# trzy/FasterRCNN

Measured on AMD Instinct MI355X. Metric: images/sec (600x1000) Faster-RCNN VGG-16 inference, higher is better.
Workload: dtype f32 (float32 tensors and accumulation; 15 GEMM layers in the f32x3 split-operand emulation = two fp16 terms per block-scaled operand, three fp16 MFMAs per product; 0 in f32x6 = three bf16 terms, six bf16 MFMAs; the other 2 on exact-f32 MFMA; strict exact-f32 everywhere: config.strict_f32_images_per_

## Files before the change

fasterrcnn_amd/_native.py:

```python
import ctypes as C
import os

_HERE = os.path.dirname(os.path.abspath(__file__))
LIB_PATH = os.environ.get("FRCNN_LIB_PATH") or os.path.join(_HERE, "csrc", "libfrcnn_hip.so")

OK = 0
ABI_VERSION = 21
ERRORS = {0: "FRCNN_OK", -1: "FRCNN_EINVAL", -2: "FRCNN_EHIP", -3: "FRCNN_ENOMEM",
          -4: "FRCNN_EUNSUPPORTED", -5: "FRCNN_ENODEVICE"}
RELU = 1
POOL2 = 2
NUM_KCLASS = 11
KCLASS_NAMES = ("conv3x3_mfma", "conv3x3_c3", "linear_mfma", "proposals", "roi_pool", "other", "winograd_transforms",
                "winograd_gemm", "winograd_x6_transforms", "winograd_x6_gemm", "winograd_x3f")

SYMBOLS = (
    "frcnn_abi_version", "frcnn_error_string", "frcnn_last_hip_error", "frcnn_device_count",
    "frcnn_anchors", "frcnn_pack_conv3x3", "frcnn_pack_conv3x3_c3", "frcnn_pack_fc_chw_to_hwc",
    "frcnn_pack_stack_rows", "frcnn_conv3x3_c3", "frcnn_conv3x3_c3_cmax", "frcnn_conv3x3_workspace_bytes", "frcnn_conv3x3_nhwc",
    "frcnn_maxpool2x2_nhwc",
    "frcnn_linear_workspace_bytes", "frcnn_linear", "frcnn_softmax_rows", "frcnn_rpn_proposals",
    "frcnn_nms", "frcnn_roi_pool", "frcnn_roi_pool_x3t", "frcnn_detections", "frcnn_ctx_create", "frcnn_ctx_create_proposals", "frcnn_ctx_destroy",
    "frcnn_ctx_bytes", "frcnn_vgg16_forward", "frcnn_ctx_tensor", "frcnn_ctx_timing_enable",
    "frcnn_ctx_timing_read",
    "frcnn_output_block_layout", "frcnn_stream_depend", "frcnn_ctx_submit_stats", "frcnn_predict_submit", "frcnn_streams_share_queue",
    "frcnn_fold_bn_pack", "frcnn_conv_workspace_bytes", "frcnn_conv_nhwc", "frcnn_conv_nhwc_math", "frcnn_conv_nhwc_x3g", "frcnn_conv_nhwc_x3g_tickets", "frcnn_pack_conv_x3g_weights", "frcnn_x3_saturation_events", "frcnn_tensor_absmax", "frcnn_conv7x7_s2_c3",
    "frcnn_maxpool3x3_s2_nhwc", "frcnn_spatial_mean_nhwc", "frcnn_resnet_forward", "frcnn_rpn_targets",
    "frcnn_preprocess_workspace_bytes", "frcnn_preprocess",
    "frcnn_conv3x3_uses_winograd", "frcnn_resnet_block_uses_winograd", "frcnn_pack_conv3x3_winograd",
    "frcnn_pack_conv3x3_winograd_taps", "frcnn_conv3x3_winograd_workspace_bytes",
    "frcnn_conv3x3_nhwc_winograd",
    "frcnn_conv3x3_uses_winograd_fused", "frcnn_resnet_block_uses_winograd_fused", "frcnn_pack_conv3x3_winograd_fused", "frcnn_pack_conv3x3_winograd_fused_taps",
    "frcnn_conv3x3_nhwc_winograd_fused",
    "frcnn_roi_align", "frcnn_roi_align_backward",
    "frcnn_x6t_record_bytes", "frcnn_split_rows_x6t", "frcnn_gemm_x6t_workspace_bytes", "frcnn_gemm_x6t", "frcnn_split_pixels_x6t", "frcnn_split_patches3x3_x6t",
    "frcnn_conv3x3_uses_winograd_x6", "frcnn_conv3x3_winograd_x6_pack_bytes", "frcnn_pack_conv3x3_winograd_x6",
    "frcnn_conv3x3_winograd_x6_workspace_bytes", "frcnn_conv3x3_nhwc_winograd_x6",
    "frcnn_pixel_absmax", "frcnn_split_pixels_x3t", "frcnn_split_patches3x3_x3t",
    "frcnn_x3t_blob_bytes", "frcnn_pack_rows_x3t", "frcnn_conv3x3_winograd_x3_pack_bytes", "frcnn_pack_conv3x3_winograd_x3",
    "frcnn_conv3x3_winograd_x3_workspace_bytes", "frcnn_conv3x3_nhwc_winograd_x3",
    "frcnn_conv3x3_winograd_x3_fused_workspace_bytes", "frcnn_conv3x3_nhwc_winograd_x3_fused", "frcnn_conv3x3_nhwc_winograd_x3_chain",
    "frcnn_x3t_record_bytes", "frcnn_rows_scale_x3t", "frcnn_split_rows_x3t", "frcnn_gemm_x3t_workspace_bytes", "frcnn_gemm_x3t",
    "frcnn_conv3x3_nhwc_winograd_fused_maps", "frcnn_ctx_create_backbone", "frcnn_resnet_backbone", "frcnn_resnet_forward_features", "frcnn_resnet_rpn_roipool", "frcnn_ctx_create_head", "frcnn_resnet_head",
    "frcnn_label_proposals", "frcnn_gather_rows", "frcnn_rpn_loss", "frcnn_detector_loss",
    "frcnn_gemm_tn_math", "frcnn_conv3x3_wgrad_math", "frcnn_conv_wgrad_math", "frcnn_bottleneck_backward_workspace_bytes", "frcnn_bottleneck_backward",
    "frcnn_gemm_tn_workspace_bytes", "frcnn_gemm_tn", "frcnn_conv3x3_wgrad_workspace_bytes", "frcnn_conv3x3_wgrad",
    "frcnn_pack_conv3x3_dgrad", "frcnn_relu_backward", "frcnn_dropout", "frcnn_dropout_relu_backward", "frcnn_add_inplace", "frcnn_maxpool2x2_backward",
    "frcnn_roi_pool_backward_workspace_bytes", "frcnn_roi_pool_backward", "frcnn_transpose", "frcnn_sgd_step", "frcnn_sgd_step_fold",
    "frcnn_conv_wgrad_workspace_bytes", "frcnn_conv_wgrad", "frcnn_conv_dgrad_workspace_bytes", "frcnn_conv_dgrad", "frcnn_conv_dgrad_math",
    "frcnn_pack_conv_dgrad", "frcnn_scale_rows", "frcnn_bn_scale_shift", "frcnn_spatial_mean_backward",
    "frcnn_ops_roi_align", "frcnn_ops_roi_align_backward", "frcnn_ops_roi_pool", "frcnn_ops_roi_pool_backward",
    "frcnn_ops_nms_workspace_bytes", "frcnn_ops_nms",
    "frcnn_ops_ms_roi_align", "frcnn_ops_ms_roi_align_workspace_bytes", "frcnn_ops_ms_roi_align_backward",
    "frcnn_ops_half_run", "frcnn_ops_roi_align_16", "frcnn_ops_roi_align_backward_16", "frcnn_ops_roi_pool_16",
    "frcnn_ops_roi_pool_backward_16", "frcnn_ops_ms_roi_align_16", "frcnn_ops_ms_roi_align_backward_16",
    "frcnn_ops_ps_roi_pool", "frcnn_ops_ps_roi_pool_backward", "frcnn_ops_ps_roi_align", "frcnn_ops_ps_roi_align_backward",
    "frcnn_ops_ps_roi_pool_16", "frcnn_ops_ps_roi_pool_backward_16", "frcnn_ops_ps_roi_align_16", "frcnn_ops_ps_roi_align_backward_16",
    "frcnn_ops_deform_workspace_bytes", "frcnn_ops_deform_forward", "frcnn_ops_deform_backward_columns", "frcnn_ops_deform_backward_offset",
    "frcnn_ops_deform_input_plan", "frcnn_ops_deform_backward_input", "frcnn_ops_deform_backward_weight",
    "frcnn_ops_deform_roi_pool_cull_list", "frcnn_ops_deform_roi_pool_workspace_bytes", "frcnn_ops_deform_roi_pool",
    "frcnn_ops_deform_roi_pool_backward", "frcnn_ops_deform_roi_pool_16", "frcnn_ops_deform_roi_pool_backward_16",
    "frcnn_ops_box_iou_rotated", "frcnn_ops_nms_rotated", "frcnn_ops_roi_align_rotated_cull_list", "frcnn_ops_roi_align_rotated",
    "frcnn_ops_roi_align_rotated_backward", "frcnn_ops_roi_align_rotated_16", "frcnn_ops_roi_align_rotated_backward_16",
    "frcnn_ops_diff_iou_rotated", "frcnn_ops_diff_iou_rotated_backward",
    "frcnn_ops_soft_nms_block_threads", "frcnn_ops_soft_nms_lds_boxes", "frcnn_ops_soft_nms_max_boxes", "frcnn_ops_soft_nms_workspace_bytes",
# ... 304 lines not shown
    "frcnn_maxpool3x3_s2_nhwc": (C.c_int, [_vp, _vp, _i, _i, _i, _vp]),
    "frcnn_spatial_mean_nhwc": (C.c_int, [_vp, _vp, _i, _i, _i, _i, _vp]),
    "frcnn_resnet_forward": (C.c_int, [_vp, C.POINTER(ResNetWeights), C.POINTER(ForwardParams), _vp, _i, _i,
                                       _vp, _vp, _vp, _vp, _vp, _vp, _vp]),
    "frcnn_resnet_forward_features": (C.c_int, [_vp, C.POINTER(ResNetWeights), C.POINTER(ForwardParams), _vp, _i, _i,
                                                _vp, _vp, _vp, _vp, _vp, _vp, _vp]),
    "frcnn_resnet_backbone": (C.c_int, [_vp, C.POINTER(ResNetWeights), C.POINTER(ForwardParams), _vp, _i, _i, _i, _vp, _vp]),
    "frcnn_pixel_absmax": (C.c_int, [_vp, _vp, C.c_longlong, _i, _vp]),
    "frcnn_split_pixels_x3t": (C.c_int, [_vp, _vp, _vp, _vp, _i, _i, _i, _i, _i, _i, _vp]),
    "frcnn_split_patches3x3_x3t": (C.c_int, [_vp, _vp, _vp, _vp, _i, _i, _i, _i, _i, _i, _vp]),
    "frcnn_x3t_blob_bytes": (C.c_size_t, [_i, _i, _i]),
    "frcnn_pack_rows_x3t": (C.c_int, [_vp, _i, _sz, _vp, _i, _i, _i, _i, _vp]),
    "frcnn_conv3x3_winograd_x3_pack_bytes": (C.c_size_t, [_i, _i]),
    "frcnn_pack_conv3x3_winograd_x3": (C.c_int, [_vp, _vp, _i, _i, _vp]),
    "frcnn_conv3x3_winograd_x3_workspace_bytes": (C.c_size_t, [_i, _i, _i, _i, _i]),
    "frcnn_conv3x3_nhwc_winograd_x3": (C.c_int, [_vp, _vp, _vp, _vp, _i, _i, _i, _i, _i, _u, _vp, _sz, _vp]),
    "frcnn_conv3x3_winograd_x3_fused_workspace_bytes": (C.c_size_t, [_i, _i, _i]),
    "frcnn_conv3x3_nhwc_winograd_x3_fused": (C.c_int, [_vp, _vp, _vp, _vp, _i, _i, _i, _i, _i, _u, _vp, _sz, _vp]),
    "frcnn_conv3x3_nhwc_winograd_x3_chain": (C.c_int, [_vp, _vp, _vp, _vp, _i, _i, _i, _i, _i, _u, _i, _vp, _sz, _vp, _vp, _vp]),
    "frcnn_x3t_record_bytes": (C.c_size_t, [_i, _i]),
    "frcnn_rows_scale_x3t": (C.c_int, [_vp, _i, _sz, _vp, _i, _i, _i, _i, _vp]),
    "frcnn_split_rows_x3t": (C.c_int, [_vp, _i, _sz, _vp, _vp, _i, _i, _i, _i, _vp]),
    "frcnn_gemm_x3t_workspace_bytes": (C.c_size_t, [_i, _i, _i, _i]),
    "frcnn_gemm_x3t": (C.c_int, [_vp, _vp, _i, _sz, _sz, _vp, _vp, _i, _sz, _sz, _vp, _vp, _vp, _i, _sz, _i, _i, _i, _i, _u, _vp, _sz, _vp]),
    "frcnn_ctx_create_backbone": (C.c_int, [C.POINTER(C.c_void_p), _i, _i, _i]),
    "frcnn_ctx_create_head": (C.c_int, [C.POINTER(C.c_void_p), _i]),
    "frcnn_resnet_rpn_roipool": (C.c_int, [_vp, C.POINTER(ResNetWeights), C.POINTER(ForwardParams), _vp, _i, _i, _vp, _vp, _vp, _vp, _vp, _vp]),
    "frcnn_resnet_head": (C.c_int, [_vp, C.POINTER(ResNetWeights), C.POINTER(ForwardParams), _vp, _i, _vp, _vp, _vp]),
    "frcnn_conv3x3_nhwc_winograd_fused_maps": (C.c_int, [_vp, _vp, _vp, _vp, _i, _i, _i, _i, _i, _u, _vp]),
    "frcnn_label_proposals": (C.c_int, [_vp, _vp, _i, _vp, _vp, _i, _i, _f, _f, C.POINTER(C.c_float), C.POINTER(C.c_float),
                                        _vp, _vp, _vp, _vp, _vp, _vp]),
    "frcnn_gather_rows": (C.c_int, [_vp, _vp, _i, _i, _vp, _vp]),
    "frcnn_rpn_loss": (C.c_int, [_vp, _i, _i, _vp, _i, _vp, _vp, _vp, _vp]),
    "frcnn_detector_loss": (C.c_int, [_vp, _vp, _vp, _vp, _i, _i, _vp, _vp, _i, _vp]),
    "frcnn_gemm_tn_workspace_bytes": (C.c_size_t, [_i, _i, _i]),
    "frcnn_gemm_tn": (C.c_int, [_vp, _i, _vp, _i, _vp, _i, _i, _i, _i, _vp, _sz, _vp]),
    "frcnn_gemm_tn_math": (C.c_int, [_vp, _i, _vp, _i, _vp, _i, _i, _i, _i, _i, _vp, _sz, _vp]),
    "frcnn_conv3x3_wgrad_math": (C.c_int, [_vp, _vp, _vp, _i, _i, _i, _i, _i, _vp, _sz, _vp]),
    "frcnn_conv_wgrad_math": (C.c_int, [_vp, _vp, _vp, _i, _i, _i, _i, _i, _i, _i, _i, _i, _vp, _sz, _vp]),
    "frcnn_bottleneck_backward_workspace_bytes": (C.c_int, [_vp, _vp, _vp, _vp, _i, _i, _i, _i, _i, C.POINTER(C.c_size_t), C.POINTER(C.c_size_t)]),
    "frcnn_bottleneck_backward": (C.c_int, [_vp, _vp, _vp, _vp, _vp, _vp, _vp, _vp, _vp, _vp, _vp, _vp, _vp, _i, _i, _i, _i, _i, _i, _vp, _sz, _vp, _sz,
                                            _vp, _vp]),
    "frcnn_conv3x3_wgrad_workspace_bytes": (C.c_size_t, [_i, _i, _i, _i]),
    "frcnn_conv3x3_wgrad": (C.c_int, [_vp, _vp, _vp, _i, _i, _i, _i, _vp, _sz, _vp]),
    "frcnn_pack_conv3x3_dgrad": (C.c_int, [_vp, _vp, _i, _i, _vp]),
    "frcnn_conv_wgrad_workspace_bytes": (C.c_size_t, [_i] * 8),
# ... 96 lines not shown
```

fasterrcnn_amd/csrc/api.hip:

```cpp
#include "common.h"
#include <algorithm>
#include <cmath>
#include <cstring>
#include <initializer_list>
#include <string>
#include <vector>
#include <new>

namespace frcnn {

static thread_local std::string g_hip_error;
void set_hip_error(hipError_t e) { g_hip_error = hipGetErrorString(e); }

static size_t align_up(size_t v, size_t a) { return (v + a - 1) / a * a; }

struct EventRec { int cls; hipEvent_t start, stop; };

struct Scratch {
    void* p = nullptr;
    size_t bytes = 0;
    int reserve(size_t want, hipStream_t s, bool zero)
    {
        if (want <= bytes) return FRCNN_OK;
        if (p) { FRCNN_HIP_TRY(hipStreamSynchronize(s)); release(); }
// ... 308 lines not shown
    if (!d_a || !d_inv_scale) return FRCNN_EINVAL;
    return launch_rows_scale_x3t(d_a, lda, a_batch_floats, d_inv_scale, rows, rows_padded, K, batches, as_stream(stream));
}

int frcnn_split_rows_x3t(const float* d_a, int lda, size_t a_batch_floats, const float* d_inv_scale, void* d_rec, int rows, int rows_padded,
                         int K, int batches, void* stream)
{
    if (!d_a || !d_rec || !d_inv_scale) return FRCNN_EINVAL;
    return launch_split_rows_x3t(d_a, lda, a_batch_floats, d_inv_scale, d_rec, rows, rows_padded, K, batches, as_stream(stream));
}

size_t frcnn_gemm_x3t_workspace_bytes(int M, int N, int K, int batches) { return gemm_x3t_workspace_bytes(M, N, K, batches); }

int frcnn_gemm_x3t(const void* d_a_rec, const float* d_a_inv, int a_rows, size_t a_batch_bytes, size_t a_inv_batch_floats,
                   const void* d_b_rec, const float* d_b_inv, int b_rows, size_t b_batch_bytes, size_t b_inv_batch_floats,
                   const float* d_bias, const float* d_residual, float* d_c, int ldc, size_t c_batch_floats, int M, int N, int K,
                   int batches, unsigned flags, void* d_ws, size_t ws_bytes, void* stream)
{
    return launch_gemm_x3t(d_a_rec, d_a_inv, a_rows, a_batch_bytes, a_inv_batch_floats, d_b_rec, d_b_inv, b_rows, b_batch_bytes,
                           b_inv_batch_floats, d_bias, d_residual, d_c, ldc, c_batch_floats, M, N, K, batches, flags, d_ws, ws_bytes,
                           as_stream(stream));
}

size_t frcnn_conv3x3_winograd_x3_fused_workspace_bytes(int n_maps, int H, int W)
{
    return n_maps > 0 && H > 0 && W > 0 ? conv3x3_winograd_x3_fused_workspace_bytes(n_maps, H, W) : 0;
}

int frcnn_conv3x3_nhwc_winograd_x3_fused(const float* d_x, const void* d_blob, const float* d_bias, float* d_y, int n_maps, int H, int W,
                                         int cin, int cout, unsigned flags, void* d_ws, size_t ws_bytes, void* stream)
{
    if (!d_x || !d_blob || !d_bias || !d_y) return FRCNN_EINVAL;
    return launch_conv3x3_winograd_x3_fused(d_x, d_blob, d_bias, d_y, n_maps, H, W, cin, cout, flags, d_ws, ws_bytes, as_stream(stream));
}

int frcnn_pixel_absmax(const float* d_x, float* d_cmax, long long pixels, int c, void* stream)
{
    if (!d_x || !d_cmax) return FRCNN_EINVAL;
    return launch_pixel_absmax(d_x, d_cmax, pixels, c, as_stream(stream));
}

int frcnn_split_pixels_x3t(const float* d_x, const float* d_cmax, void* d_rec, float* d_inv_scale, int n_maps, int H, int W, int c, int stride,
                           int rows_padded, void* stream)
{
    if (!d_x || !d_rec) return FRCNN_EINVAL;
    return launch_split_pixels_x3t(d_x, d_cmax, d_rec, d_inv_scale, n_maps, H, W, c, stride, rows_padded, as_stream(stream));
// ... 1582 lines not shown
```

fasterrcnn_amd/csrc/common.h:

```cpp
#pragma once
#include <hip/hip_runtime.h>
#include <stdint.h>
#include <stddef.h>
#include <stdlib.h>
#include "../../include/frcnn_hip.h"

typedef float f32x4  __attribute__((ext_vector_type(4)));
typedef float f32x16 __attribute__((ext_vector_type(16)));

inline const char* frcnn_knob(const char* name)
{
#ifdef FRCNN_EXPERIMENT_KNOBS
    return getenv(name);
#else
    (void)name;
    return nullptr;
#endif
}

namespace frcnn {

void set_hip_error(hipError_t e);

inline int check_launch() {
// ... 108 lines not shown
size_t gemm_x6t_workspace_bytes(int M, int N, int K, int batches);
void gemm_x6t_set_tiles(int mode);
int launch_gemm_x6t(const void* a_rec, int a_rows, size_t a_batch_bytes, const void* b_rec, int b_rows, size_t b_batch_bytes,
                    const float* bias, const float* residual, float* c, int ldc, size_t c_batch_floats, int M, int N, int K, int batches,
                    unsigned flags, void* ws, size_t ws_bytes, hipStream_t s, int tiles_mode = -1);
int launch_split_pixels_x6t(const float* x, void* rec, int N, int H, int W, int C, int stride, int rows_padded, hipStream_t s);
int gemm_x6t_get_tiles();
int launch_gemm_x6t_reduce(const float* ws, const float* bias, const float* residual, float* c, int ldc, size_t c_batch_floats, int M, int N,
                           int batches, int splits, int relu, hipStream_t s);
size_t x3t_record_bytes(int rows_padded, int K);
int launch_rows_scale_x3t(const float* a, int lda, size_t a_batch_floats, float* inv_scale, int R, int rows_padded, int K, int batches,
                          hipStream_t s);
int launch_split_rows_x3t(const float* a, int lda, size_t a_batch_floats, const float* inv_scale, void* rec, int R, int rows_padded, int K,
                          int batches, hipStream_t s);
int launch_split_pixels_x3t(const float* x, const float* cmax, void* rec, float* inv, int N, int H, int W, int C, int stride, int rows_padded,
                            hipStream_t s);
int launch_split_patches3x3_x3t(const float* x, const float* cmax, void* rec, float* inv, int N, int H, int W, int C, int stride,
                                int rows_padded, hipStream_t s);
size_t gemm_x3t_workspace_bytes(int M, int N, int K, int batches);
int launch_gemm_x3t(const void* a_rec, const float* a_inv, int a_rows, size_t a_batch_bytes, size_t a_inv_batch, const void* b_rec,
                    const float* b_inv, int b_rows, size_t b_batch_bytes, size_t b_inv_batch, const float* bias, const float* residual,
                    float* c, int ldc, size_t c_batch_floats, int M, int N, int K, int batches, unsigned flags, void* ws, size_t ws_bytes,
                    hipStream_t s, int tiles_mode = -1);
size_t x3t_blob_bytes(int rows_padded, int K, int batches);
int launch_pack_rows_x3t(const float* a, int lda, size_t a_batch_floats, void* blob, int R, int rows_padded, int K, int batches, hipStream_t s);
int launch_pixel_absmax(const float* x, float* cmax, long long pixels, int C, hipStream_t s);
size_t conv3x3_winograd_x3_pack_bytes(int cout, int cin);
int launch_pack_conv3x3_winograd_x3(const float* u_f32, void* ublob, int cout, int cin, hipStream_t s);
size_t conv3x3_winograd_x3_workspace_bytes(int N, int H, int W, int cin, int cout);
int winograd_x3_plan(int N, int H, int W, int cin, int cout, unsigned flags, void* ws, size_t ws_bytes, void** V, float** vinv, float** cmax,
                     float** M, void** G, size_t* g_bytes);
int launch_winograd_x3_input(const float* x, float* cmax, void* vrec, float* vinv, int N, int H, int W, int cin, hipStream_t s,
                             const float* cmax_ready = nullptr);
int launch_winograd_x3_gemm(const void* vrec, const float* vinv, const void* ublob, float* M, int N, int H, int W, int cin, int cout, void* gws,
                            size_t gws_bytes, hipStream_t s);
int launch_conv3x3_winograd_x3(const float* x, const void* ublob, const float* b, float* y, int N, int H, int W, int cin, int cout,
                               unsigned flags, void* ws, size_t ws_bytes, hipStream_t s,
                               const float* cmax_ready = nullptr, float* cmax_out = nullptr);
size_t conv3x3_winograd_x3_fused_workspace_bytes(int N, int H, int W);
int launch_conv3x3_winograd_x3_fused(const float* x, const void* ublob, const float* b, float* y, int N, int H, int W, int cin, int cout,
                                     unsigned flags, void* ws, size_t ws_bytes, hipStream_t s, const float* cmax_ready = nullptr,
                                     float* cmax_out = nullptr);
int launch_roi_pool_x3t(const float* fm, int fh, int fw, int c, const float* rois, const int32_t* n_rois, int max_rois, int pooled,
                        float scale, float* cmax, float* inv, void* rec, int rec_rows, hipStream_t s, bool cmax_ready = false);
bool conv3x3_uses_winograd_x6(int cin, int cout);
size_t conv3x3_winograd_x6_pack_bytes(int cout, int cin);
// ... 98 lines not shown
```

fasterrcnn_amd/csrc/gemm_x3t.hip:

```cpp
#include "x3t.h"

namespace frcnn {

typedef _Float16 hx_f16x8 __attribute__((ext_vector_type(8)));

#ifndef HX_ABLATE
#define HX_ABLATE 0
#endif
__global__ __launch_bounds__(256)
void rows_scale_x3t_kernel(const float* __restrict__ a, int lda, size_t a_batch, float* __restrict__ inv_scale, int R, int rows_padded,
                           int K, int batches)
{
    const int lane = threadIdx.x & 63;
    const long long wave = (long long)blockIdx.x * 4 + (threadIdx.x >> 6);
    if (wave >= (long long)batches * rows_padded) return;
    const int row = (int)(wave % rows_padded), batch = (int)(wave / rows_padded);
    float mx = 0.f;
    if (row < R) {
        const float* src = a + (size_t)batch * a_batch + (size_t)row * lda;
        for (int k = 4 * lane; k < K; k += 256) {
            const f32x4 v = *reinterpret_cast<const f32x4*>(src + k);
            mx = fmaxf(fmaxf(mx, fmaxf(fabsf(v[0]), fabsf(v[1]))), fmaxf(fabsf(v[2]), fabsf(v[3])));
        }
    }
// ... 162 lines not shown
    *reinterpret_cast<uint4*>(dst) = ph;
    *reinterpret_cast<uint4*>(dst + HX_PIECE) = pl;
}

struct HxParams {
    const unsigned char* a;
    const unsigned char* b;
    const float* a_inv;
    const float* b_inv;
    float* c;
    float* ws;
    const float* bias;
    const float* residual;
    size_t a_batch, b_batch, c_batch;
    size_t a_inv_batch, b_inv_batch;
    int a_rbt, b_rbt;
    int M, N, ldc;
    int nchunks, chunks_per_split, splits, batches;
    int mtiles, ntiles;
    int relu;
    int total;
};

template <int WTM, int WTN, int WVM, int WVN, int NSUB>
struct HxCfg {
    static constexpr int NW = WVM * WVN, THREADS = 64 * NW;
    static constexpr int ARB = WVM * WTM, BRB = WVN * WTN;
    static constexpr int BM = 32 * ARB, BN = 32 * BRB;
    static constexpr int A_BYTES = ARB * HX_RB, B_BYTES = BRB * HX_RB;
    static constexpr int STAGE1 = A_BYTES + B_BYTES;
    static constexpr int STAGE = NSUB * STAGE1;
    static constexpr int NBUF = NSUB == 1 ? 3 : 2;
    static constexpr int DIST = NBUF - 1;
    static constexpr size_t LDS_BYTES = NBUF * (size_t)STAGE;
    static constexpr int NPA = ARB * 2, NPB = BRB * 2, NP = NPA + NPB;
    static constexpr int PPW = (NSUB * NP + NW - 1) / NW;
};

typedef __attribute__((address_space(3))) void* hx_lds_ptr;

template <int WTM, int WTN, int WVM, int WVN, int NSUB>
__global__ __launch_bounds__(64 * WVM * WVN, 2)
void gemm_x3t_kernel(const HxParams p)
{
    using C = HxCfg<WTM, WTN, WVM, WVN, NSUB>;
    extern __shared__ __attribute__((aligned(16))) unsigned char smem_hx[];
    const int tid = threadIdx.x, lane = tid & 63;
    const int wave = __builtin_amdgcn_readfirstlane(tid >> 6);
    const int wm = wave / WVN, wn = wave % WVN;

    int bid = blockIdx.x;
    {
        const int q = p.total >> 3, r = p.total & 7, xcd = bid & 7, idx = bid >> 3;
        bid = (xcd < r ? xcd * (q + 1) : r * (q + 1) + (xcd - r) * q) + idx;
    }
    const int nt = bid % p.ntiles;
    int t = bid / p.ntiles;
    const int mt = t % p.mtiles;
    t /= p.mtiles;
    const int split = t % p.splits;
    const int batch = t / p.splits;

    const int c_begin = split * p.chunks_per_split;
    int c_end = c_begin + p.chunks_per_split;
    if (c_end > p.nchunks) c_end = p.nchunks;
    const int nst = (c_end - c_begin) / NSUB;

    const size_t a_chunk = (size_t)p.a_rbt * HX_RB, b_chunk = (size_t)p.b_rbt * HX_RB;
// ... 24 lines not shown
    hx_f16x8 ah[WTM], al[WTM], bh[WTN], bl[WTN];
#pragma unroll
    for (int i = 0; i < WTM; ++i)
#pragma unroll
        for (int e = 0; e < 8; ++e) al[i][e] = (_Float16)0.f;
#pragma unroll
    for (int j = 0; j < WTN; ++j)
#pragma unroll
        for (int e = 0; e < 8; ++e) bh[j][e] = (_Float16)0.f;

#ifndef HX_NO_SCHED
#define HX_NO_SCHED 0
#endif
#define HX_SGB(mask, n) __builtin_amdgcn_sched_group_barrier(mask, n, 0)
#define HX_TERM(A, B)                                                                                  \
    _Pragma("unroll") for (int i = 0; i < WTM; ++i)                                                     \
        _Pragma("unroll") for (int j = 0; j < WTN; ++j)                                                 \
            if (!(HX_ABLATE & 2)) acc[i][j] = __builtin_amdgcn_mfma_f32_32x32x16_f16(B[j], A[i], acc[i][j], 0, 0, 0);

#ifdef HX_CLOCKS
    unsigned long long clk0 = 0, real0 = 0, clk1 = 0, real1 = 0;
    const unsigned long long real_entry = __builtin_amdgcn_s_memrealtime();
#endif
    if (nst > 0) {
        issue_stage(0, 0);
        if (C::DIST == 2) issue_stage(nst > 1 ? 1 : 0, 1);
        asm volatile("s_waitcnt vmcnt(%0)" ::"n"((C::DIST - 1) * C::PPW) : "memory");
        __builtin_amdgcn_s_barrier();
        int cur = 0;
        const int a_off = wm * WTM * HX_RB + lane * 16;
        const int b_off = C::A_BYTES + wn * WTN * HX_RB + lane * 16;
#ifdef HX_CLOCKS
        clk0 = __builtin_readcyclecounter(); real0 = __builtin_amdgcn_s_memrealtime();
#endif
        for (int s = 0; s < nst; ++s) {
            const int nxt = C::NBUF == 3 ? (cur == 0 ? 2 : cur - 1) : (cur ^ 1);
#pragma unroll
            for (int sub = 0; sub < NSUB; ++sub) {
                const unsigned char* at = smem_hx + cur * C::STAGE + sub * C::STAGE1 + a_off;
                const unsigned char* bt = smem_hx + cur * C::STAGE + sub * C::STAGE1 + b_off;
                if (!(HX_ABLATE & 16) || s == 0) {
#pragma unroll
                for (int i = 0; i < WTM; ++i) ah[i] = *reinterpret_cast<const hx_f16x8*>(at + i * HX_RB);
#pragma unroll
                for (int j = 0; j < WTN; ++j) bl[j] = *reinterpret_cast<const hx_f16x8*>(bt + j * HX_RB + HX_PIECE);
                }
// ... 151 lines not shown
    HxPlan pl;
    const int chunks = K / 16;
    static const int env_force = []() { const char* e = frcnn_knob("FRCNN_HX_CFG"); return e ? atoi(e) : -1; }();
    const int mode = tiles_mode >= 0 ? tiles_mode : gemm_x6t_get_tiles();
    const int force = (env_force >= 0 && tiles_mode < 0) ? env_force : (mode == 1 ? 0 : mode == 2 ? 1 : -1);
    const long long u0 = (long long)cdiv(M, 320) * cdiv(N, 256) * batches;
    const long long u1 = (long long)cdiv(M, 160) * cdiv(N, 128) * batches;
    int splits0 = 1;
    while (u0 * splits0 * 2 <= 256 && chunks / (splits0 * 2) >= 8) splits0 *= 2;
    const double c0 = (double)((u0 * splits0 + 255) / 256) * 1920.0 / splits0 + (splits0 > 1 ? 600.0 : 0.0);
    int splits1 = 1;
    while (u1 * splits1 * 2 <= 256 && chunks / (splits1 * 2) >= 8) splits1 *= 2;
    const double c1 = (double)((u1 * splits1 + 255) / 256) * 480.0 / 0.85 / splits1 + (splits1 > 1 ? 600.0 : 0.0);
    pl.cfg = (force == 0 || force == 1) ? force : (c1 < c0 ? 1 : 0);
    static const bool big_unsplit = frcnn_knob("FRCNN_HX_BIG_UNSPLIT") != nullptr;
    if (big_unsplit && force < 0 && pl.cfg == 1 && splits1 == 1) { pl.cfg = 0; splits0 = 1; }
    int splits = pl.cfg == 1 ? splits1 : splits0;
    if (splits > chunks) splits = chunks;
    pl.mtiles = pl.cfg == 1 ? cdiv(M, 160) : cdiv(M, 320);
    pl.ntiles = pl.cfg == 1 ? cdiv(N, 128) : cdiv(N, 256);
    pl.chunks_per_split = cdiv(chunks, splits);
    pl.splits = cdiv(chunks, pl.chunks_per_split);
    return pl;
}

size_t gemm_x3t_workspace_bytes(int M, int N, int K, int batches)
{
    if (!gemm_x6t_shape_ok(M, N, K, batches)) return 0;
    size_t need = 0;
    for (int mode = 0; mode < 3; ++mode) {
        const HxPlan pl = plan_gemm_x3t(M, N, K, batches, mode);
        const size_t b = pl.splits > 1 ? (size_t)pl.splits * batches * M * N * sizeof(float) : 0;
        if (b > need) need = b;
    }
    return need;
}

int launch_gemm_x3t(const void* a_rec, const float* a_inv, int a_rows, size_t a_batch_bytes, size_t a_inv_batch, const void* b_rec,
                    const float* b_inv, int b_rows, size_t b_batch_bytes, size_t b_inv_batch, const float* bias, const float* residual,
                    float* c, int ldc, size_t c_batch_floats, int M, int N, int K, int batches, unsigned flags, void* ws, size_t ws_bytes,
                    hipStream_t s, int tiles_mode)
{
    if (!gemm_x6t_shape_ok(M, N, K, batches)) return FRCNN_EUNSUPPORTED;
    if (!a_rec || !b_rec || !a_inv || !b_inv || !c || a_rows % 320 != 0 || a_rows < M || b_rows % 256 != 0 || b_rows < N || ldc < N ||
        ldc % 4 != 0)
        return FRCNN_EINVAL;
    const HxPlan pl = plan_gemm_x3t(M, N, K, batches, tiles_mode);
    if (pl.splits > 1 && (ws == nullptr || ws_bytes < (size_t)pl.splits * batches * M * N * sizeof(float))) return FRCNN_EINVAL;
    HxParams p;
    p.a = static_cast<const unsigned char*>(a_rec);
    p.b = static_cast<const unsigned char*>(b_rec);
    p.a_inv = a_inv; p.b_inv = b_inv;
    p.c = c;
    p.ws = static_cast<float*>(ws);
    p.bias = bias;
    p.residual = residual;
    p.a_batch = a_batch_bytes; p.b_batch = b_batch_bytes; p.c_batch = c_batch_floats;
    p.a_inv_batch = a_inv_batch; p.b_inv_batch = b_inv_batch;
    p.a_rbt = a_rows / 32; p.b_rbt = b_rows / 32;
    p.M = M; p.N = N; p.ldc = ldc;
    p.nchunks = K / 16; p.chunks_per_split = pl.chunks_per_split; p.splits = pl.splits; p.batches = batches;
    p.mtiles = pl.mtiles; p.ntiles = pl.ntiles;
    p.relu = (flags & FRCNN_RELU) ? 1 : 0;
    const long long total = (long long)pl.mtiles * pl.ntiles * batches * pl.splits;
    if (total > 0x7fffffffLL) return FRCNN_EINVAL;
    p.total = (int)total;
    static const int env_nsub = []() { const char* e = frcnn_knob("FRCNN_HX_NSUB"); return e ? atoi(e) : 0; }();
    const int last = p.nchunks - (pl.splits - 1) * pl.chunks_per_split;
    const bool even = pl.chunks_per_split % 2 == 0 && last % 2 == 0;
    const int nsub = !even ? 1 : (env_nsub == 1 || env_nsub == 2) ? env_nsub : (pl.chunks_per_split >= 64 ? 2 : 1);
#define HX_LAUNCH(TM, TN, VM, VN, NS)                                                                          \
    do {                                                                                                      \
        using C = HxCfg<TM, TN, VM, VN, NS>;                                                                    \
        auto kern = gemm_x3t_kernel<TM, TN, VM, VN, NS>;                                                        \
        FRCNN_MAX_LDS_ONCE(kern, C::LDS_BYTES);                                                                 \
        hipLaunchKernelGGL(kern, dim3((unsigned)total), dim3(C::THREADS), C::LDS_BYTES, s, p);                  \
    } while (0)
    if (pl.cfg == 1) { if (nsub == 2) HX_LAUNCH(5, 1, 1, 4, 2); else HX_LAUNCH(5, 1, 1, 4, 1); }
    else             { if (nsub == 2) HX_LAUNCH(5, 2, 2, 4, 2); else HX_LAUNCH(5, 2, 2, 4, 1); }
#undef HX_LAUNCH
    int rc = check_launch();
    if (rc || pl.splits == 1) return rc;
    return launch_gemm_x6t_reduce(static_cast<const float*>(ws), bias, residual, c, ldc, c_batch_floats, M, N, batches, pl.splits, p.relu, s);
}

}
```

include/frcnn_hip.h:

```cpp
#ifndef FRCNN_HIP_H
#define FRCNN_HIP_H

#include <stddef.h>
#include <stdint.h>

#ifdef __cplusplus
extern "C" {
#endif

#define FRCNN_OK            0
#define FRCNN_EINVAL       -1
#define FRCNN_EHIP         -2
#define FRCNN_ENOMEM       -3
#define FRCNN_EUNSUPPORTED -4
#define FRCNN_ENODEVICE    -5

#define FRCNN_ABI_VERSION 21

#define FRCNN_RELU   1u
#define FRCNN_POOL2  2u
#define FRCNN_X3G_WSPLIT 0x800u

int         frcnn_abi_version(void);
const char* frcnn_error_string(int code);
// ... 64 lines not shown
int frcnn_pack_rows_x3t(const float* d_a, int lda, size_t a_batch_floats, void* d_blob, int rows, int rows_padded, int K, int batches,
                        void* stream);
size_t frcnn_conv3x3_winograd_x3_pack_bytes(int cout, int cin);
int frcnn_pack_conv3x3_winograd_x3(const float* d_u_f32, void* d_blob, int cout, int cin, void* stream);
size_t frcnn_conv3x3_winograd_x3_workspace_bytes(int n_maps, int H, int W, int cin, int cout);
int frcnn_conv3x3_nhwc_winograd_x3(const float* d_x, const void* d_blob, const float* d_bias, float* d_y, int n_maps, int H, int W, int cin,
                                   int cout, unsigned flags, void* d_ws, size_t ws_bytes, void* stream);
size_t frcnn_conv3x3_winograd_x3_fused_workspace_bytes(int n_maps, int H, int W);
int frcnn_conv3x3_nhwc_winograd_x3_fused(const float* d_x, const void* d_blob, const float* d_bias, float* d_y, int n_maps, int H, int W,
                                         int cin, int cout, unsigned flags, void* d_ws, size_t ws_bytes, void* stream);
int frcnn_conv3x3_nhwc_winograd_x3_chain(const float* d_x, const void* d_blob, const float* d_bias, float* d_y, int n_maps, int H, int W, int cin,
                                         int cout, unsigned flags, int one_launch, void* d_ws, size_t ws_bytes, const float* d_cmax_in,
                                         float* d_cmax_out, void* stream);
size_t frcnn_x3t_record_bytes(int rows_padded, int K);
int frcnn_rows_scale_x3t(const float* d_a, int lda, size_t a_batch_floats, float* d_inv_scale, int rows, int rows_padded, int K, int batches,
                         void* stream);
int frcnn_split_rows_x3t(const float* d_a, int lda, size_t a_batch_floats, const float* d_inv_scale, void* d_rec, int rows, int rows_padded,
                         int K, int batches, void* stream);
size_t frcnn_gemm_x3t_workspace_bytes(int M, int N, int K, int batches);
int frcnn_gemm_x3t(const void* d_a_rec, const float* d_a_inv, int a_rows, size_t a_batch_bytes, size_t a_inv_batch_floats,
                   const void* d_b_rec, const float* d_b_inv, int b_rows, size_t b_batch_bytes, size_t b_inv_batch_floats,
                   const float* d_bias, const float* d_residual, float* d_c, int ldc, size_t c_batch_floats, int M, int N, int K,
                   int batches, unsigned flags, void* d_ws, size_t ws_bytes, void* stream);

int frcnn_split_pixels_x6t(const float* d_x, void* d_rec, int N, int H, int W, int C, int stride, int rows_padded, void* stream);
int frcnn_conv3x3_uses_winograd_x6(int cin, int cout);
size_t frcnn_conv3x3_winograd_x6_pack_bytes(int cout, int cin);
int frcnn_pack_conv3x3_winograd_x6(const float* d_w_oihw, const float* d_row_scale, void* d_u_rec, int cout, int cin, void* stream);
size_t frcnn_conv3x3_winograd_x6_workspace_bytes(int n_maps, int H, int W, int cin, int cout);
int frcnn_conv3x3_nhwc_winograd_x6(const float* d_x, const void* d_u_rec, const float* d_bias, float* d_y, int n_maps, int H, int W, int cin,
                                   int cout, unsigned flags, void* d_ws, size_t ws_bytes, void* stream);
int frcnn_split_patches3x3_x6t(const float* d_x, void* d_rec, int N, int H, int W, int C, int stride, int rows_padded, void* stream);
int frcnn_maxpool2x2_nhwc(const float* d_x, float* d_y, int H, int W, int c, void* stream);

int frcnn_fold_bn_pack(const float* d_w_oihw, const float* d_gamma, const float* d_beta,
                       const float* d_mean, const float* d_var, float eps, int cout, int cin, int ksize,
                       float* d_w_packed, float* d_b_packed, void* stream);
size_t frcnn_conv_workspace_bytes(int N, int H, int W, int cin, int cout, int ksize, int stride, int pad);
int frcnn_conv_nhwc(const float* d_x, const float* d_w_packed, const float* d_bias, const float* d_residual,
                    float* d_y, int N, int H, int W, int cin, int cout, int ksize, int stride, int pad,
                    unsigned flags, void* d_ws, size_t ws_bytes, void* stream);
int frcnn_conv7x7_s2_c3(const float* d_x_chw, const float* d_w_packed, const float* d_bias, float* d_y,
                        int H, int W, int cout, unsigned flags, void* stream);
int frcnn_maxpool3x3_s2_nhwc(const float* d_x, float* d_y, int H, int W, int c, void* stream);
int frcnn_spatial_mean_nhwc(const float* d_x, float* d_y, int N, int H, int W, int c, void* stream);

// ... 499 lines not shown
```

Measured before the change: 980.9.

## Load x3t GEMM B operand directly into registers instead of staging through LDS

Adds a BREG variant of the x3t split-fp16 GEMM kernel. B fragments are fetched with buffer loads straight into registers, double-buffered per sub-chunk, and only A is staged in LDS with a configurable buffer depth. This variant is selected by default for the main tile config when the two-sub-chunk path applies. The aim is to cut LDS traffic, LDS footprint and the LDS read latency on B, at the cost of more VGPRs, uncoalesced-per-wave global reads of B, and a hand-tuned waitcnt and schedule scheme. It also adds API hooks to force the form and query the selection.

```diff
diff --git a/fasterrcnn_amd/_native.py b/fasterrcnn_amd/_native.py
--- a/fasterrcnn_amd/_native.py
+++ b/fasterrcnn_amd/_native.py
@@ -41,6 +41,7 @@
     "frcnn_conv3x3_winograd_x3_workspace_bytes", "frcnn_conv3x3_nhwc_winograd_x3",
     "frcnn_conv3x3_winograd_x3_fused_workspace_bytes", "frcnn_conv3x3_nhwc_winograd_x3_fused", "frcnn_conv3x3_nhwc_winograd_x3_chain",
     "frcnn_x3t_record_bytes", "frcnn_rows_scale_x3t", "frcnn_split_rows_x3t", "frcnn_gemm_x3t_workspace_bytes", "frcnn_gemm_x3t",
+    "frcnn_gemm_x3t_set_form", "frcnn_gemm_x3t_form",
     "frcnn_conv3x3_nhwc_winograd_fused_maps", "frcnn_ctx_create_backbone", "frcnn_resnet_backbone", "frcnn_resnet_forward_features", "frcnn_resnet_rpn_roipool", "frcnn_ctx_create_head", "frcnn_resnet_head",
     "frcnn_label_proposals", "frcnn_gather_rows", "frcnn_rpn_loss", "frcnn_detector_loss",
     "frcnn_gemm_tn_math", "frcnn_conv3x3_wgrad_math", "frcnn_conv_wgrad_math", "frcnn_bottleneck_backward_workspace_bytes", "frcnn_bottleneck_backward",
@@ -391,6 +392,8 @@
     "frcnn_rows_scale_x3t": (C.c_int, [_vp, _i, _sz, _vp, _i, _i, _i, _i, _vp]),
     "frcnn_split_rows_x3t": (C.c_int, [_vp, _i, _sz, _vp, _vp, _i, _i, _i, _i, _vp]),
     "frcnn_gemm_x3t_workspace_bytes": (C.c_size_t, [_i, _i, _i, _i]),
+    "frcnn_gemm_x3t_set_form": (None, [_i, _i]),
+    "frcnn_gemm_x3t_form": (C.c_int, [_i, _i, _i, _i, _i, _i]),
     "frcnn_gemm_x3t": (C.c_int, [_vp, _vp, _i, _sz, _sz, _vp, _vp, _i, _sz, _sz, _vp, _vp, _vp, _i, _sz, _i, _i, _i, _i, _u, _vp, _sz, _vp]),
     "frcnn_ctx_create_backbone": (C.c_int, [C.POINTER(C.c_void_p), _i, _i, _i]),
     "frcnn_ctx_create_head": (C.c_int, [C.POINTER(C.c_void_p), _i]),
diff --git a/fasterrcnn_amd/csrc/api.hip b/fasterrcnn_amd/csrc/api.hip
--- a/fasterrcnn_amd/csrc/api.hip
+++ b/fasterrcnn_amd/csrc/api.hip
@@ -354,6 +354,14 @@
                            as_stream(stream));
 }
 
+void frcnn_gemm_x3t_set_form(int form, int tiles)
+{
+    gemm_x3t_set_form(form);
+    gemm_x6t_set_tiles(tiles == 1 || tiles == 2 ? tiles : 0);
+}
+
+int frcnn_gemm_x3t_form(int M, int N, int K, int batches, int a_rows, int b_rows) { return gemm_x3t_form(M, N, K, batches, a_rows, b_rows); }
+
 size_t frcnn_conv3x3_winograd_x3_fused_workspace_bytes(int n_maps, int H, int W)
 {
     return n_maps > 0 && H > 0 && W > 0 ? conv3x3_winograd_x3_fused_workspace_bytes(n_maps, H, W) : 0;
diff --git a/fasterrcnn_amd/csrc/common.h b/fasterrcnn_amd/csrc/common.h
--- a/fasterrcnn_amd/csrc/common.h
+++ b/fasterrcnn_amd/csrc/common.h
@@ -154,6 +154,9 @@
                     const float* b_inv, int b_rows, size_t b_batch_bytes, size_t b_inv_batch, const float* bias, const float* residual,
                     float* c, int ldc, size_t c_batch_floats, int M, int N, int K, int batches, unsigned flags, void* ws, size_t ws_bytes,
                     hipStream_t s, int tiles_mode = -1);
+enum { HX_FORM_LDS = 1, HX_FORM_BREG = 2 };
+void gemm_x3t_set_form(int form);
+int gemm_x3t_form(int M, int N, int K, int batches, int a_rows, int b_rows);
 size_t x3t_blob_bytes(int rows_padded, int K, int batches);
 int launch_pack_rows_x3t(const float* a, int lda, size_t a_batch_floats, void* blob, int R, int rows_padded, int K, int batches, hipStream_t s);
 int launch_pixel_absmax(const float* x, float* cmax, long long pixels, int C, hipStream_t s);
diff --git a/fasterrcnn_amd/csrc/gemm_x3t.hip b/fasterrcnn_amd/csrc/gemm_x3t.hip
--- a/fasterrcnn_amd/csrc/gemm_x3t.hip
+++ b/fasterrcnn_amd/csrc/gemm_x3t.hip
@@ -208,28 +208,35 @@
     int total;
 };
 
-template <int WTM, int WTN, int WVM, int WVN, int NSUB>
+#ifndef HX_BREG_NBUF
+#define HX_BREG_NBUF 3
+#endif
+#ifndef HX_BREG_B_AUX
+#define HX_BREG_B_AUX 0
+#endif
+template <int WTM, int WTN, int WVM, int WVN, int NSUB, bool BREG = false>
 struct HxCfg {
     static constexpr int NW = WVM * WVN, THREADS = 64 * NW;
     static constexpr int ARB = WVM * WTM, BRB = WVN * WTN;
     static constexpr int BM = 32 * ARB, BN = 32 * BRB;
     static constexpr int A_BYTES = ARB * HX_RB, B_BYTES = BRB * HX_RB;
-    static constexpr int STAGE1 = A_BYTES + B_BYTES;
+    static constexpr int STAGE1 = A_BYTES + (BREG ? 0 : B_BYTES);
     static constexpr int STAGE = NSUB * STAGE1;
-    static constexpr int NBUF = NSUB == 1 ? 3 : 2;
+    static constexpr int NBUF = BREG ? HX_BREG_NBUF : NSUB == 1 ? 3 : 2;
     static constexpr int DIST = NBUF - 1;
     static constexpr size_t LDS_BYTES = NBUF * (size_t)STAGE;
-    static constexpr int NPA = ARB * 2, NPB = BRB * 2, NP = NPA + NPB;
+    static constexpr int NPA = ARB * 2, NPB = BREG ? 0 : BRB * 2, NP = NPA + NPB;
     static constexpr int PPW = (NSUB * NP + NW - 1) / NW;
+    static constexpr int BLW = 2 * NSUB * WTN;
 };
 
 typedef __attribute__((address_space(3))) void* hx_lds_ptr;
 
-template <int WTM, int WTN, int WVM, int WVN, int NSUB>
+template <int WTM, int WTN, int WVM, int WVN, int NSUB, bool BREG = false>
 __global__ __launch_bounds__(64 * WVM * WVN, 2)
 void gemm_x3t_kernel(const HxParams p)
 {
-    using C = HxCfg<WTM, WTN, WVM, WVN, NSUB>;
+    using C = HxCfg<WTM, WTN, WVM, WVN, NSUB, BREG>;
     extern __shared__ __attribute__((aligned(16))) unsigned char smem_hx[];
     const int tid = threadIdx.x, lane = tid & 63;
     const int wave = __builtin_amdgcn_readfirstlane(tid >> 6);
@@ -300,6 +307,125 @@
     unsigned long long clk0 = 0, real0 = 0, clk1 = 0, real1 = 0;
     const unsigned long long real_entry = __builtin_amdgcn_s_memrealtime();
 #endif
+    if constexpr (BREG) {
+        static_assert(NSUB == 2 && (NSUB * C::NPA) % C::NW == 0 && C::BLW + C::PPW <= 63, "whole pieces per wave; the stage's loads fit vmcnt");
+        static_assert(C::DIST >= 2, "the A pieces of stage s + 1 are older than stage s's own loads");
+        const int nch = c_end - c_begin;
+        const int nsta = (nch + 1) >> 1;
+        const int lane16 = lane * 16, b_chunk_i = (int)b_chunk;
+        const __amdgpu_buffer_rsrc_t brs = __builtin_amdgcn_make_buffer_rsrc(
+            const_cast<unsigned char*>(p.b + (size_t)batch * p.b_batch + (size_t)nt * C::B_BYTES + (size_t)c_begin * b_chunk + wn * WTN * HX_RB), 0,
+            (nch - 1) * b_chunk_i + WTN * HX_RB, 0x00020000);
+        auto load_b = [&](int ch, int j, int term) -> hx_f16x8 {
+            ch = ch < nch ? ch : nch - 1;
+            return __builtin_bit_cast(hx_f16x8, __builtin_amdgcn_raw_buffer_load_b128(brs, lane16 + j * HX_RB + term * HX_PIECE, ch * b_chunk_i, HX_BREG_B_AUX));
+        };
+        const int a_chunk_i = (int)a_chunk;
+        const __amdgpu_buffer_rsrc_t ars = __builtin_amdgcn_make_buffer_rsrc(
+            const_cast<unsigned char*>(p.a + (size_t)batch * p.a_batch + (size_t)mt * C::A_BYTES + (size_t)c_begin * a_chunk), 0,
+            (nch - 1) * a_chunk_i + C::A_BYTES, 0x00020000);
+        auto issue_a = [&](int s, int buf) {
+            unsigned char* ldsb = smem_hx + buf * C::STAGE;
+#pragma unroll
+            for (int i = 0; i < C::PPW; ++i) {
+                const int q = wave + C::NW * i, sub = q / C::NPA, r = q - sub * C::NPA;
+                int ch = s * NSUB + sub;
+                ch = ch < nch ? ch : nch - 1;
+                __builtin_amdgcn_raw_ptr_buffer_load_lds(ars, (hx_lds_ptr)(ldsb + sub * C::STAGE1 + r * HX_PIECE), 16, lane16, ch * a_chunk_i + r * HX_PIECE, 0, 0);
+            }
+        };
+#define HX_TERMB(A, B)                                                                                 \
+    _Pragma("unroll") for (int i = 0; i < WTM; ++i)                                                     \
+        _Pragma("unroll") for (int j = 0; j < WTN; ++j) {                                               \
+            if (!(HX_ABLATE & 2)) acc[i][j] = __builtin_amdgcn_mfma_f32_32x32x16_f16(B[j], A[i], acc[i][j], 0, 0, 0); \
+            else if (i == 0) asm volatile("" ::"v"(B[j]));                                              \
+        }
+        hx_f16x8 bhr[2][WTN], blr[2][WTN];
+#pragma unroll
+        for (int j = 0; j < WTN; ++j) {
+#pragma unroll
+            for (int e = 0; e < 8; ++e) bhr[1][j][e] = (_Float16)0.f;
+            bhr[0][j] = load_b(0, j, 0);
+            blr[0][j] = load_b(0, j, 1);
+            blr[1][j] = load_b(1, j, 1);
+        }
+#pragma unroll
+        for (int d = 0; d < C::DIST; ++d) issue_a(d < nsta ? d : nsta - 1, d);
+        asm volatile("s_waitcnt vmcnt(%0)" ::"n"((C::DIST - 1) * C::PPW) : "memory");
+        __builtin_amdgcn_s_barrier();
+        int cur = 0;
+        const int a_off = wm * WTM * HX_RB + lane * 16;
+#ifdef HX_CLOCKS
+        clk0 = __builtin_readcyclecounter(); real0 = __builtin_amdgcn_s_memrealtime();
+#endif
+        for (int s = 0; s < nst; ++s) {
+            const int nxt = cur == 0 ? C::NBUF - 1 : cur - 1;
+#pragma unroll
+            for (int sub = 0; sub < NSUB; ++sub) {
+                const unsigned char* at = smem_hx + cur * C::STAGE + sub * C::STAGE1 + a_off;
+                const int c = s * NSUB + sub;
+                if (!(HX_ABLATE & 16) || s == 0) {
+#pragma unroll
+                for (int i = 0; i < WTM; ++i) ah[i] = *reinterpret_cast<const hx_f16x8*>(at + i * HX_RB);
+                }
+                if (sub == 0 && !(HX_ABLATE & 1)) issue_a(s + C::DIST < nsta ? s + C::DIST : nsta - 1, nxt);
+                HX_TERMB(al, bhr[sub ^ 1])
+                if (!(HX_ABLATE & 8)) {
+#pragma unroll
+                for (int j = 0; j < WTN; ++j) bhr[sub ^ 1][j] = load_b(c + 1, j, 0);
+                }
+                HX_TERMB(ah, blr[sub])
+                if (!(HX_ABLATE & 8)) {
+#pragma unroll
+                for (int j = 0; j < WTN; ++j) blr[sub][j] = load_b(c + 2, j, 1);
+                }
+                if (!(HX_ABLATE & 16) || s == 0) {
+#pragma unroll
+                for (int i = 0; i < WTM; ++i) al[i] = *reinterpret_cast<const hx_f16x8*>(at + i * HX_RB + HX_PIECE);
+                }
+                HX_TERMB(ah, bhr[sub])
+#if !HX_NO_SCHED && !HX_ABLATE
+                constexpr int NT = WTM * WTN, PW = C::PPW;
+                HX_SGB(0x100, WTM);
+                if (sub == 0) {
+                    _Pragma("unroll") for (int q = 0; q < (PW < NT ? PW : NT); ++q) { HX_SGB(0x008, 1); HX_SGB(0x010, 1); }
+                    if (PW > NT) HX_SGB(0x010, PW - NT);
+                    if (NT > PW) HX_SGB(0x008, NT - PW);
+                } else {
+                    HX_SGB(0x008, NT);
+                }
+                HX_SGB(0x010, WTN);
+                _Pragma("unroll") for (int q = 0; q < (WTM < NT ? WTM : NT); ++q) { HX_SGB(0x008, 1); HX_SGB(0x100, 1); }
+                if (NT > WTM) HX_SGB(0x008, NT - WTM);
+                HX_SGB(0x010, WTN);
+                HX_SGB(0x008, NT);
+#endif
+            }
+            __builtin_amdgcn_sched_barrier(0);
+            asm volatile("s_waitcnt vmcnt(%0) lgkmcnt(0)" ::"n"(C::PPW + C::BLW) : "memory");
+            __builtin_amdgcn_s_barrier();
+            cur = cur == C::NBUF - 1 ? 0 : cur + 1;
+            __builtin_amdgcn_sched_barrier(0);
+        }
+#ifdef HX_CLOCKS
+        clk1 = __builtin_readcyclecounter(); real1 = __builtin_amdgcn_s_memrealtime();
+#endif
+        if (nch & 1) {
+            const unsigned char* at = smem_hx + cur * C::STAGE + a_off;
+#pragma unroll
+            for (int i = 0; i < WTM; ++i) ah[i] = *reinterpret_cast<const hx_f16x8*>(at + i * HX_RB);
+            HX_TERMB(al, bhr[1])
+            HX_TERMB(ah, blr[0])
+#pragma unroll
+            for (int i = 0; i < WTM; ++i) al[i] = *reinterpret_cast<const hx_f16x8*>(at + i * HX_RB + HX_PIECE);
+            HX_TERMB(ah, bhr[0])
+#pragma unroll
+            for (int j = 0; j < WTN; ++j) bhr[1][j] = bhr[0][j];
+        }
+        HX_TERMB(al, bhr[1])
+#undef HX_TERMB
+        asm volatile("s_waitcnt vmcnt(0)" ::: "memory");
+    } else
     if (nst > 0) {
         issue_stage(0, 0);
         if (C::DIST == 2) issue_stage(nst > 1 ? 1 : 0, 1);
@@ -497,6 +623,34 @@
     pl.chunks_per_split = cdiv(chunks, splits);
     pl.splits = cdiv(chunks, pl.chunks_per_split);
     return pl;
+}
+
+#ifndef HX_BREG_DEFAULT
+#define HX_BREG_DEFAULT 1
+#endif
+static thread_local int g_hx_form = 0;
+void gemm_x3t_set_form(int form) { g_hx_form = form == HX_FORM_LDS || form == HX_FORM_BREG ? form : 0; }
+
+static int hx_nsub(const HxPlan& pl, int nchunks)
+{
+    static const int env_nsub = []() { const char* e = frcnn_knob("FRCNN_HX_NSUB"); return e ? atoi(e) : 0; }();
+    const int last = nchunks - (pl.splits - 1) * pl.chunks_per_split;
+    const bool even = pl.chunks_per_split % 2 == 0 && last % 2 == 0;
+    return !even ? 1 : (env_nsub == 1 || env_nsub == 2) ? env_nsub : (pl.chunks_per_split >= 64 ? 2 : 1);
+}
+
+static int hx_form(const HxPlan& pl, int nchunks, int a_rows, int b_rows)
+{
+    const size_t rows = (size_t)(a_rows > b_rows ? a_rows : b_rows);
+    const bool can = pl.cfg == 0 && (size_t)pl.chunks_per_split * (rows / 32) * HX_RB <= 0x7fffffffu;
+    const bool want = g_hx_form == HX_FORM_BREG || (g_hx_form == 0 && HX_BREG_DEFAULT && hx_nsub(pl, nchunks) == 2);
+    return can && want ? HX_FORM_BREG : HX_FORM_LDS;
+}
+
+int gemm_x3t_form(int M, int N, int K, int batches, int a_rows, int b_rows)
+{
+    if (!gemm_x6t_shape_ok(M, N, K, batches) || a_rows % 320 != 0 || a_rows < M || b_rows % 256 != 0 || b_rows < N) return 0;
+    return hx_form(plan_gemm_x3t(M, N, K, batches), K / 16, a_rows, b_rows);
 }
 
 size_t gemm_x3t_workspace_bytes(int M, int N, int K, int batches)
@@ -540,19 +694,17 @@
     const long long total = (long long)pl.mtiles * pl.ntiles * batches * pl.splits;
     if (total > 0x7fffffffLL) return FRCNN_EINVAL;
     p.total = (int)total;
-    static const int env_nsub = []() { const char* e = frcnn_knob("FRCNN_HX_NSUB"); return e ? atoi(e) : 0; }();
-    const int last = p.nchunks - (pl.splits - 1) * pl.chunks_per_split;
-    const bool even = pl.chunks_per_split % 2 == 0 && last % 2 == 0;
-    const int nsub = !even ? 1 : (env_nsub == 1 || env_nsub == 2) ? env_nsub : (pl.chunks_per_split >= 64 ? 2 : 1);
-#define HX_LAUNCH(TM, TN, VM, VN, NS)                                                                          \
+    const int nsub = hx_nsub(pl, p.nchunks);
+#define HX_LAUNCH(TM, TN, VM, VN, NS, BR)                                                                      \
     do {                                                                                                      \
-        using C = HxCfg<TM, TN, VM, VN, NS>;                                                                    \
-        auto kern = gemm_x3t_kernel<TM, TN, VM, VN, NS>;                                                        \
+        using C = HxCfg<TM, TN, VM, VN, NS, BR>;                                                                \
+        auto kern = gemm_x3t_kernel<TM, TN, VM, VN, NS, BR>;                                                    \
         FRCNN_MAX_LDS_ONCE(kern, C::LDS_BYTES);                                                                 \
         hipLaunchKernelGGL(kern, dim3((unsigned)total), dim3(C::THREADS), C::LDS_BYTES, s, p);                  \
     } while (0)
-    if (pl.cfg == 1) { if (nsub == 2) HX_LAUNCH(5, 1, 1, 4, 2); else HX_LAUNCH(5, 1, 1, 4, 1); }
-    else             { if (nsub == 2) HX_LAUNCH(5, 2, 2, 4, 2); else HX_LAUNCH(5, 2, 2, 4, 1); }
+    if (pl.cfg == 1) { if (nsub == 2) HX_LAUNCH(5, 1, 1, 4, 2, false); else HX_LAUNCH(5, 1, 1, 4, 1, false); }
+    else if (hx_form(pl, p.nchunks, a_rows, b_rows) == HX_FORM_BREG) HX_LAUNCH(5, 2, 2, 4, 2, true);
+    else             { if (nsub == 2) HX_LAUNCH(5, 2, 2, 4, 2, false); else HX_LAUNCH(5, 2, 2, 4, 1, false); }
 #undef HX_LAUNCH
     int rc = check_launch();
     if (rc || pl.splits == 1) return rc;
diff --git a/include/frcnn_hip.h b/include/frcnn_hip.h
--- a/include/frcnn_hip.h
+++ b/include/frcnn_hip.h
@@ -110,6 +110,8 @@
                    const void* d_b_rec, const float* d_b_inv, int b_rows, size_t b_batch_bytes, size_t b_inv_batch_floats,
                    const float* d_bias, const float* d_residual, float* d_c, int ldc, size_t c_batch_floats, int M, int N, int K,
                    int batches, unsigned flags, void* d_ws, size_t ws_bytes, void* stream);
+void frcnn_gemm_x3t_set_form(int form, int tiles);
+int frcnn_gemm_x3t_form(int M, int N, int K, int batches, int a_rows, int b_rows);
 
 int frcnn_split_pixels_x6t(const float* d_x, void* d_rec, int N, int H, int W, int C, int stride, int rows_padded, void* stream);
 int frcnn_conv3x3_uses_winograd_x6(int cin, int cout);
```

After: 990.1, median of 6. No clear change (+0.9%).
